# psweens/VAN-GAN

Hardware: AMD Instinct MI355X
Metric: train Mvoxels/s (VanGan.train_step, 128^3 bf16) (higher is better)
Workload: dtype bf16; 1 GPU; VanGan.train_step, 128x128x128 volumes, batch 1 per GPU (global 1), clDice on, disc noise+dropout on; parallelism=dp1

## Files before the change

### van_gan_amd/csrc/vg_loss.hip

```cpp
#include "vg_common.h"

static inline int lblocks(int64_t n, int per = 256) { int64_t b = (n + per - 1) / per; return (int)(b > 4095 ? 4095 : (b < 1 ? 1 : b)); }

__device__ __forceinline__ float block_sum(float v, float* sm) {
    v = wave_sum(v);
    const int lane = threadIdx.x & 63, wv = threadIdx.x >> 6;
    __syncthreads();
    if (lane == 0) sm[wv] = v;
    __syncthreads();
    float r = 0.f;
    for (int i = 0; i < (int)(blockDim.x >> 6); ++i) r += sm[i];
    return r;
}

__global__ void mm_init_kernel(float* mm4, int B) {
    const int b = blockIdx.x * blockDim.x + threadIdx.x;
    if (b < B) { mm4[b * 4] = INFINITY; mm4[b * 4 + 1] = -INFINITY; mm4[b * 4 + 2] = 0.f; mm4[b * 4 + 3] = 0.f; }
}
__device__ __forceinline__ void atomic_min_f(float* a, float v) {
    unsigned* ua = (unsigned*)a; unsigned old = *ua;
    while (v < __uint_as_float(old)) { const unsigned prev = atomicCAS(ua, old, __float_as_uint(v)); if (prev == old) break; old = prev; }
}
__device__ __forceinline__ void atomic_max_f(float* a, float v) {
    unsigned* ua = (unsigned*)a; unsigned old = *ua;
// ... 139 lines not shown
    if (threadIdx.x == 0) atomicAdd(acc, s);
}
extern "C" int vg_mse(const float* a, const float* b, int64_t n, float* acc, float gscale, float* gb, int accumulate,
                      vg_stream_t stream) {
    vg_begin();
    if (!a || !b || !acc || n < 1) return VG_EINVAL;
    hipLaunchKernelGGL(mse_kernel, dim3(lblocks(n, 1024) > 511 ? 511 : lblocks(n, 1024)), dim3(256), 0, (hipStream_t)stream, a, b, n, acc, gscale, gb,
                       accumulate);
    return vg_check_launch();
}
__global__ void mse_const_kernel(const void* x, int x_f32, float target, int64_t n, float* acc, float gscale, float* gx, int accum) {
    __shared__ float sm[4];
    float s = 0.f;
    for (int64_t i = (int64_t)blockIdx.x * blockDim.x + threadIdx.x; i < n; i += (int64_t)gridDim.x * blockDim.x) {
        const float v = x_f32 ? ((const float*)x)[i] : bf2f(((const bf16_t*)x)[i]);
        const float d = v - target;
        s += d * d;
        if (gx) { const float g = gscale * 2.f * d; gx[i] = accum ? gx[i] + g : g; }
    }
    s = block_sum(s, sm);
    if (threadIdx.x == 0) atomicAdd(acc, s);
}
extern "C" int vg_mse_const(const void* x, int x_f32, float target, int64_t n, float* acc, float gscale, float* gx,
                            int accumulate, vg_stream_t stream) {
    vg_begin();
    if (!x || !acc || n < 1) return VG_EINVAL;
    hipLaunchKernelGGL(mse_const_kernel, dim3(lblocks(n, 1024)), dim3(256), 0, (hipStream_t)stream, x, x_f32, target, n, acc,
                       gscale, gx, accumulate);
    return vg_check_launch();
}
template <int P>
__device__ __forceinline__ float lp_term(float d, float gscale, float& g) {
    if (P == 1) { g = d > 0.f ? gscale : (d < 0.f ? -gscale : 0.f); return fabsf(d); }
    if (P == 2) { g = gscale * 2.f * d; return d * d; }
    const float d2 = d * d;
    g = gscale * 4.f * (d2 * d);
    return d2 * d2;
}
template <int P>
__global__ __launch_bounds__(256) void lp_loss_kernel(const float* __restrict__ a, const float* __restrict__ b, int64_t n, float* acc, float gscale,
                                                      float* gb, int accum) {
    __shared__ float sm[4];
    float s = 0.f;
    const int64_t n4 = ((((uintptr_t)a | (uintptr_t)b | (uintptr_t)gb) & 15) == 0) ? n >> 2 : 0;
    for (int64_t i = (int64_t)blockIdx.x * blockDim.x + threadIdx.x; i < n4; i += (int64_t)gridDim.x * blockDim.x) {
        const f32x4 x = ((const f32x4*)a)[i], y = ((const f32x4*)b)[i];
        f32x4 g;
#pragma unroll
        for (int j = 0; j < 4; ++j) { float gj; s += lp_term<P>(y[j] - x[j], gscale, gj); g[j] = gj; }
        if (gb) { if (accum) g += ((const f32x4*)gb)[i]; ((f32x4*)gb)[i] = g; }
    }
    for (int64_t i = 4 * n4 + (int64_t)blockIdx.x * blockDim.x + threadIdx.x; i < n; i += (int64_t)gridDim.x * blockDim.x) {
        float g;
        s += lp_term<P>(b[i] - a[i], gscale, g);
        if (gb) gb[i] = accum ? gb[i] + g : g;
    }
    s = block_sum(s, sm);
    if (threadIdx.x == 0) atomicAdd(acc, s);
}
extern "C" int vg_lp_loss(const float* a, const float* b, int64_t n, int p, float* acc, float gscale, float* gb, int accumulate,
                          vg_stream_t stream) {
    vg_begin();
    if (!a || !b || !acc || n < 1 || (p != 1 && p != 2 && p != 4)) return VG_EINVAL;
    const dim3 grid(lblocks(n, 4096) > 511 ? 511 : lblocks(n, 4096));
    hipStream_t s = (hipStream_t)stream;
    if (p == 1) hipLaunchKernelGGL(lp_loss_kernel<1>, grid, dim3(256), 0, s, a, b, n, acc, gscale, gb, accumulate);
    else if (p == 2) hipLaunchKernelGGL(lp_loss_kernel<2>, grid, dim3(256), 0, s, a, b, n, acc, gscale, gb, accumulate);
    else hipLaunchKernelGGL(lp_loss_kernel<4>, grid, dim3(256), 0, s, a, b, n, acc, gscale, gb, accumulate);
    return vg_check_launch();
}
template <int KIND>
__device__ __forceinline__ float logit_term(float x, bool one, float& g) {
    const float e = expf(-fabsf(x));
    const float r = 1.f / (1.f + e);
    const float s = x >= 0.f ? r : e * r, c = x >= 0.f ? e * r : r;
    const float l1p = log1pf(e);
    const float sp = one ? fmaxf(-x, 0.f) + l1p : fmaxf(x, 0.f) + l1p;
    if (KIND == 0) { g = one ? -c : s; return sp; }
    if (one) { g = -(c * c * c) - 2.f * s * c * c * sp; return c * c * sp; }
    g = s * s * s + 2.f * s * s * c * sp;
    return s * s * sp;
}
template <int KIND, typename T>
__global__ __launch_bounds__(256) void logit_loss_kernel(const T* __restrict__ x, int one, int64_t n, float* acc, float gscale, float* gx, int accum) {
    __shared__ float sm[4];
    float s = 0.f;
    const int64_t n8 = ((((uintptr_t)x | (uintptr_t)gx) & 15) == 0) ? n >> 3 : 0;
    for (int64_t i = (int64_t)blockIdx.x * blockDim.x + threadIdx.x; i < n8; i += (int64_t)gridDim.x * blockDim.x) {
        float v[8], g[8];
        load8<T>(x + 8 * i, v);
#pragma unroll
        for (int j = 0; j < 8; ++j) { s += logit_term<KIND>(v[j], one != 0, g[j]); g[j] *= gscale; }
        if (gx) {
            if (accum) {
                float o[8]; load8<float>(gx + 8 * i, o);
#pragma unroll
                for (int j = 0; j < 8; ++j) g[j] += o[j];
            }
            store8<float>(gx + 8 * i, g);
        }
    }
    for (int64_t i = 8 * n8 + (int64_t)blockIdx.x * blockDim.x + threadIdx.x; i < n; i += (int64_t)gridDim.x * blockDim.x) {
        float g;
        s += logit_term<KIND>(ld1<T>(x + i), one != 0, g);
        g *= gscale;
        if (gx) gx[i] = accum ? gx[i] + g : g;
    }
    s = block_sum(s, sm);
    if (threadIdx.x == 0) atomicAdd(acc, s);
}
extern "C" int vg_logit_loss(const void* x, int x_f32, float target, int kind, int64_t n, float* acc, float gscale, float* gx,
                             int accumulate, vg_stream_t stream) {
    vg_begin();
    if (!x || !acc || n < 1 || (target != 0.f && target != 1.f) || (kind != 0 && kind != 1)) return VG_EINVAL;
    const dim3 grid(lblocks(n, 2048) > 255 ? 255 : lblocks(n, 2048));
    hipStream_t s = (hipStream_t)stream;
    const int one = target == 1.f;
#define VG_LOGIT_LAUNCH(K, T) hipLaunchKernelGGL((logit_loss_kernel<K, T>), grid, dim3(256), 0, s, (const T*)x, one, n, acc, gscale, gx, accumulate)
    if (kind == 0) { if (x_f32) VG_LOGIT_LAUNCH(0, float); else VG_LOGIT_LAUNCH(0, bf16_t); }
    else           { if (x_f32) VG_LOGIT_LAUNCH(1, float); else VG_LOGIT_LAUNCH(1, bf16_t); }
#undef VG_LOGIT_LAUNCH
    return vg_check_launch();
}
__global__ void dot_sums_kernel(const float* a, const float* b, int64_t n, float* sums3) {
    __shared__ float sm[4];
    float s0 = 0.f, s1 = 0.f, s2 = 0.f;
    const int64_t n4 = ((((uintptr_t)a | (uintptr_t)b) & 15) == 0) ? n >> 2 : 0;
    for (int64_t i = (int64_t)blockIdx.x * blockDim.x + threadIdx.x; i < n4; i += (int64_t)gridDim.x * blockDim.x) {
        const f32x4 x = ((const f32x4*)a)[i], y = ((const f32x4*)b)[i];
#pragma unroll
        for (int j = 0; j < 4; ++j) { s0 += x[j] * y[j]; s1 += x[j]; s2 += y[j]; }
    }
    for (int64_t i = 4 * n4 + (int64_t)blockIdx.x * blockDim.x + threadIdx.x; i < n; i += (int64_t)gridDim.x * blockDim.x) {
        const float x = a[i], y = b[i]; s0 += x * y; s1 += x; s2 += y;
    }
    s0 = block_sum(s0, sm); s1 = block_sum(s1, sm); s2 = block_sum(s2, sm);
    if (threadIdx.x == 0) { atomicAdd(&sums3[0], s0); atomicAdd(&sums3[1], s1); atomicAdd(&sums3[2], s2); }
}
extern "C" int vg_dot_sums(const float* a, const float* b, int64_t n, float* sums3, vg_stream_t stream) {
    vg_begin();
    if (!a || !b || !sums3 || n < 1) return VG_EINVAL;
    const int blocks = lblocks(n, 4096) > 255 ? 255 : lblocks(n, 4096);
    hipLaunchKernelGGL(dot_sums_kernel, dim3(blocks), dim3(256), 0, (hipStream_t)stream, a, b, n, sums3);
    return vg_check_launch();
}

__device__ __forceinline__ void gauss3(float* g) {
    const float e = expf(-0.5f * (1.f / 1.5f) * (1.f / 1.5f));
    const float s = 1.f + 2.f * e;
    g[0] = e / s; g[1] = 1.f / s; g[2] = e / s;
}
#define SSIM_C1 1e-4f
#define SSIM_C2 9e-4f
__global__ void ssim_fwd_kernel(const float* t, const float* p, int B, int D, int H, int W, float* acc, float* part) {
    __shared__ float sm[4];
    float g[3]; gauss3(g);
    const int64_t S = (int64_t)D * H * W, total = (int64_t)B * S;
    float loss = 0.f;
    for (int64_t i = (int64_t)blockIdx.x * blockDim.x + threadIdx.x; i < total; i += (int64_t)gridDim.x * blockDim.x) {
        const int w = (int)(i % W); int64_t r = i / W; const int h = (int)(r % H); r /= H; const int d = (int)(r % D); const int b = (int)(r / D);
        float mt = 0.f, mp = 0.f, ett = 0.f, epp = 0.f, etp = 0.f;
        for (int a = -1; a <= 1; ++a) { const int dd = d + a; if (dd < 0 || dd >= D) continue;
            for (int c = -1; c <= 1; ++c) { const int hh = h + c; if (hh < 0 || hh >= H) continue;
                for (int e = -1; e <= 1; ++e) { const int ww = w + e; if (ww < 0 || ww >= W) continue;
                    const float wt = g[a + 1] * g[c + 1] * g[e + 1];
                    const size_t j = (size_t)b * S + ((size_t)dd * H + hh) * W + ww;
                    const float tv = t[j], pv = p[j];
                    mt += wt * tv; mp += wt * pv; ett += wt * tv * tv; epp += wt * pv * pv; etp += wt * tv * pv;
                } } }
        const float stt = ett - mt * mt, spp = epp - mp * mp, stp = etp - mt * mp;
        const float A = 2.f * mt * mp + SSIM_C1, Bq = 2.f * stp + SSIM_C2;
        const float Cq = mt * mt + mp * mp + SSIM_C1, Dq = stt + spp + SSIM_C2;
        const float inv = 1.f / (Cq * Dq);
        const float ssim = A * Bq * inv;
        loss += 1.f - ssim;
        if (part) {
            const float dmu = (2.f * mt * Bq - 2.f * mt * A) * inv - ssim * (2.f * mp * Dq - 2.f * mp * Cq) * inv;
            const float depp = -ssim / Dq;
            const float detp = 2.f * A * inv;
            part[i] = -dmu; part[total + i] = -depp; part[2 * total + i] = -detp;
        }
    }
    loss = block_sum(loss, sm);
    if (threadIdx.x == 0) atomicAdd(acc, loss);
}
extern "C" int vg_ssim_fwd(const float* t, const float* p, int B, int D, int H, int W, float* acc, float* part,
                           vg_stream_t stream) {
    vg_begin();
    if (!t || !p || !acc || B < 1 || D < 1 || H < 1 || W < 1) return VG_EINVAL;
    const int blocks = lblocks((int64_t)B * D * H * W) > 1023 ? 1023 : lblocks((int64_t)B * D * H * W);
    hipLaunchKernelGGL(ssim_fwd_kernel, dim3(blocks), dim3(256), 0, (hipStream_t)stream, t, p, B, D, H, W, acc, part);
    return vg_check_launch();
}
__global__ void ssim_bwd_kernel(const float* t, const float* p, const float* part, int B, int D, int H, int W, float gscale,
                                float* gp, int accum) {
    float g[3]; gauss3(g);
    const int64_t S = (int64_t)D * H * W, total = (int64_t)B * S;
    for (int64_t i = (int64_t)blockIdx.x * blockDim.x + threadIdx.x; i < total; i += (int64_t)gridDim.x * blockDim.x) {
        const int w = (int)(i % W); int64_t r = i / W; const int h = (int)(r % H); r /= H; const int d = (int)(r % D); const int b = (int)(r / D);
        float f0 = 0.f, f1 = 0.f, f2 = 0.f;
        for (int a = -1; a <= 1; ++a) { const int dd = d + a; if (dd < 0 || dd >= D) continue;
            for (int c = -1; c <= 1; ++c) { const int hh = h + c; if (hh < 0 || hh >= H) continue;
                for (int e = -1; e <= 1; ++e) { const int ww = w + e; if (ww < 0 || ww >= W) continue;
                    const float wt = g[a + 1] * g[c + 1] * g[e + 1];
                    const size_t j = (size_t)b * S + ((size_t)dd * H + hh) * W + ww;
                    f0 += wt * part[j]; f1 += wt * part[total + j]; f2 += wt * part[2 * total + j];
                } } }
        const float v = gscale * (f0 + 2.f * p[i] * f1 + t[i] * f2);
        gp[i] = accum ? gp[i] + v : v;
    }
}
extern "C" int vg_ssim_bwd(const float* t, const float* p, const float* part, int B, int D, int H, int W, float gscale,
                           float* gp, int accumulate, vg_stream_t stream) {
    vg_begin();
    if (!t || !p || !part || !gp || B < 1) return VG_EINVAL;
    hipLaunchKernelGGL(ssim_bwd_kernel, dim3(lblocks((int64_t)B * D * H * W)), dim3(256), 0, (hipStream_t)stream, t, p, part, B, D, H, W,
                       gscale, gp, accumulate);
    return vg_check_launch();
}

#define SK_TW 32
#define SK_TH 8
#define SK_TD 8
template <bool ERODE>
__global__ __launch_bounds__(256) void skel_tile_kernel(const float* __restrict__ in, const float* __restrict__ imgj,
                                                        const float* __restrict__ prev, int D, int H, int W, float* __restrict__ out) {
    __shared__ float t[SK_TD + 2][SK_TH + 2][SK_TW + 2];
    const int tid = threadIdx.x;
    const int tiles_w = (W + SK_TW - 1) / SK_TW, tiles_h = (H + SK_TH - 1) / SK_TH;
    int bt = blockIdx.x;
    const int tw = bt % tiles_w; bt /= tiles_w;
    const int th = bt % tiles_h; const int td = bt / tiles_h;
    const int w0 = tw * SK_TW, h0 = th * SK_TH, d0 = td * SK_TD;
    const size_t vol = (size_t)blockIdx.y * D * H * W;
    const float fill = ERODE ? INFINITY : -INFINITY;
    constexpr int NH = (SK_TD + 2) * (SK_TH + 2) * (SK_TW + 2);
    for (int i = tid; i < NH; i += 256) {
        const int x = i % (SK_TW + 2); const int r = i / (SK_TW + 2);
        const int y = r % (SK_TH + 2), z = r / (SK_TH + 2);
        const int gw = w0 + x - 1, gh = h0 + y - 1, gd = d0 + z - 1;
        float v = fill;
        if (gw >= 0 && gw < W && gh >= 0 && gh < H && gd >= 0 && gd < D) v = in[vol + ((size_t)gd * H + gh) * W + gw];
        (&t[0][0][0])[i] = v;
    }
    __syncthreads();
    const int tx = tid & (SK_TW - 1), ty = tid >> 5;
    const int gw = w0 + tx, gh = h0 + ty;
    float p9[3], p5[3];
#pragma unroll
    for (int sl = 0; sl < SK_TD + 2; ++sl) {
        const float a00 = t[sl][ty][tx], a01 = t[sl][ty][tx + 1], a02 = t[sl][ty][tx + 2];
        const float a10 = t[sl][ty + 1][tx], a11 = t[sl][ty + 1][tx + 1], a12 = t[sl][ty + 1][tx + 2];
        const float a20 = t[sl][ty + 2][tx], a21 = t[sl][ty + 2][tx + 1], a22 = t[sl][ty + 2][tx + 2];
        float plus, full;
        if (ERODE) {
            plus = fminf(fminf(fminf(a01, a21), fminf(a10, a12)), a11);
            full = fminf(plus, fminf(fminf(a00, a02), fminf(a20, a22)));
        } else {
            plus = fmaxf(fmaxf(fmaxf(a01, a21), fmaxf(a10, a12)), a11);
            full = fmaxf(plus, fmaxf(fmaxf(a00, a02), fmaxf(a20, a22)));
        }
        p9[sl % 3] = full; p5[sl % 3] = plus;
        if (sl >= 2) {
            const int gd = d0 + sl - 2;
            const int c = (sl - 1) % 3, lo = (sl - 2) % 3, hi = sl % 3;
            const float nb = ERODE ? fminf(p9[c], fminf(p5[lo], p5[hi])) : fmaxf(p9[c], fmaxf(p9[lo], p9[hi]));
            if (gw < W && gh < H && gd < D) {
                const size_t o = vol + ((size_t)gd * H + gh) * W + gw;
                if (ERODE) out[o] = nb;
                else {
                    const float delta = fmaxf(imgj[o] - nb, 0.f);
                    if (prev) { const float sp = prev[o]; out[o] = sp + fmaxf(delta - sp * delta, 0.f); }
                    else out[o] = delta;
                }
            }
        }
    }
}
template <bool AUX>
__global__ __launch_bounds__(256) void skel_chain_kernel(const float* __restrict__ imgs, int64_t n, int iters, int D, int H, int W,
                                                         float* __restrict__ skels, float* __restrict__ deltas, unsigned char* __restrict__ codes) {
    __shared__ float t[SK_TD + 2][SK_TH + 2][SK_TW + 2];
    const int tid = threadIdx.x;
    const int tiles_w = (W + SK_TW - 1) / SK_TW, tiles_h = (H + SK_TH - 1) / SK_TH;
    int bt = blockIdx.x;
    const int tw = bt % tiles_w; bt /= tiles_w;
    const int th = bt % tiles_h; const int td = bt / tiles_h;
    const int w0 = tw * SK_TW, h0 = th * SK_TH, d0 = td * SK_TD;
    const size_t vol = (size_t)blockIdx.y * D * H * W;
    constexpr int NH = (SK_TD + 2) * (SK_TH + 2) * (SK_TW + 2);
    const int tx = tid & (SK_TW - 1), ty = tid >> 5;
    const int gw = w0 + tx, gh = h0 + ty;
    const bool col_ok = gw < W && gh < H;
    float cen[SK_TD], sk[SK_TD];
#pragma unroll
    for (int k = 0; k < SK_TD; ++k) {
        const int gd = d0 + k;
        cen[k] = (col_ok && gd < D) ? imgs[vol + ((size_t)gd * H + gh) * W + gw] : 0.f;
        sk[k] = 0.f;
    }
    for (int j = 0; j <= iters; ++j) {
        const float* __restrict__ in = imgs + (size_t)(j + 1) * n;
        __syncthreads();
        for (int i = tid; i < NH; i += 256) {
            const int x = i % (SK_TW + 2); const int r = i / (SK_TW + 2);
            const int y = r % (SK_TH + 2), z = r / (SK_TH + 2);
            const int qw = w0 + x - 1, qh = h0 + y - 1, qd = d0 + z - 1;
            float v = -INFINITY;
            if (qw >= 0 && qw < W && qh >= 0 && qh < H && qd >= 0 && qd < D) v = in[vol + ((size_t)qd * H + qh) * W + qw];
            (&t[0][0][0])[i] = v;
        }
        __syncthreads();
        float* __restrict__ out = skels + (size_t)j * n;
        float p9[3]; int k9[3];
#pragma unroll
        for (int sl = 0; sl < SK_TD + 2; ++sl) {
            const float a00 = t[sl][ty][tx], a01 = t[sl][ty][tx + 1], a02 = t[sl][ty][tx + 2];
            const float a10 = t[sl][ty + 1][tx], a11 = t[sl][ty + 1][tx + 1], a12 = t[sl][ty + 1][tx + 2];
            const float a20 = t[sl][ty + 2][tx], a21 = t[sl][ty + 2][tx + 1], a22 = t[sl][ty + 2][tx + 2];
            if (AUX) {
                float m = a00; int k = 0;
                if (a01 > m) { m = a01; k = 1; } if (a02 > m) { m = a02; k = 2; }
                if (a10 > m) { m = a10; k = 3; } if (a11 > m) { m = a11; k = 4; } if (a12 > m) { m = a12; k = 5; }
                if (a20 > m) { m = a20; k = 6; } if (a21 > m) { m = a21; k = 7; } if (a22 > m) { m = a22; k = 8; }
                p9[sl % 3] = m; k9[sl % 3] = k;
            } else {
                const float plus = fmaxf(fmaxf(fmaxf(a01, a21), fmaxf(a10, a12)), a11);
                p9[sl % 3] = fmaxf(plus, fmaxf(fmaxf(a00, a02), fmaxf(a20, a22)));
            }
            if (sl >= 2) {
                const int k = sl - 2, gd = d0 + k;
                const float nb = fmaxf(p9[(sl - 1) % 3], fmaxf(p9[(sl - 2) % 3], p9[sl % 3]));
                const float delta = fmaxf(cen[k] - nb, 0.f);
                const float sp = sk[k];
                sk[k] = j ? sp + fmaxf(delta - sp * delta, 0.f) : delta;
                if (col_ok && gd < D) {
                    const size_t o = vol + ((size_t)gd * H + gh) * W + gw;
                    out[o] = sk[k];
                    if (AUX) {
                        float best = p9[(sl - 2) % 3]; int code = k9[(sl - 2) % 3];
                        if (p9[(sl - 1) % 3] > best) { best = p9[(sl - 1) % 3]; code = 9 + k9[(sl - 1) % 3]; }
                        if (p9[sl % 3] > best) { best = p9[sl % 3]; code = 18 + k9[sl % 3]; }
                        deltas[(size_t)j * n + o] = delta; codes[(size_t)j * n + o] = (unsigned char)code;
                    }
                }
            }
        }
#pragma unroll
        for (int k = 0; k < SK_TD; ++k) cen[k] = t[k + 1][ty + 1][tx + 1];
    }
}
__device__ __forceinline__ int64_t sk_off(int code, int H, int W) {
    const int a = code / 9, r = code - a * 9, b = r / 3, c = r - b * 3;
    return ((int64_t)(a - 1) * H + (b - 1)) * W + (c - 1);
}
#define SK_TILE_ORIGIN()                                                                                    \
    const int tiles_w = (W + SK_TW - 1) / SK_TW, tiles_h = (H + SK_TH - 1) / SK_TH;                           \
    int bt_ = blockIdx.x; const int tw_ = bt_ % tiles_w; bt_ /= tiles_w;                                      \
    const int th_ = bt_ % tiles_h, td_ = bt_ / tiles_h;                                                       \
    const int w0 = tw_ * SK_TW, h0 = th_ * SK_TH, d0 = td_ * SK_TD;                                           \
    const size_t vol = (size_t)blockIdx.y * D * H * W;                                                        \
    const int tx = tid & (SK_TW - 1), ty = tid >> 5; const int gw = w0 + tx, gh = h0 + ty;

template <int E>
__device__ __forceinline__ void erode_stage(const float* __restrict__ src, float* __restrict__ dst, int w0, int h0, int d0, int D, int H, int W,
                                            size_t vol, float* __restrict__ out, int tid) {
    constexpr int DD = SK_TD + 2 * E, DH = SK_TH + 2 * E, DW = SK_TW + 2 * E;
    constexpr int SH = DH + 2, SW = DW + 2;
    for (int col = tid; col < DH * DW; col += 256) {
        const int y = col / DW, x = col - y * DW;
        const int gh = h0 - E + y, gw = w0 - E + x;
        const bool col_in = gh >= 0 && gh < H && gw >= 0 && gw < W;
        const bool col_tile = y >= E && y < E + SK_TH && x >= E && x < E + SK_TW;
        float p9[3], p5[3];
#pragma unroll
        for (int sl = 0; sl < DD + 2; ++sl) {
            const float* r0 = src + (sl * SH + y) * SW + x;
            const float* r1 = r0 + SW; const float* r2 = r1 + SW;
            const float a00 = r0[0], a01 = r0[1], a02 = r0[2], a10 = r1[0], a11 = r1[1], a12 = r1[2], a20 = r2[0], a21 = r2[1], a22 = r2[2];
            const float plus = fminf(fminf(fminf(a01, a21), fminf(a10, a12)), a11);
            p9[sl % 3] = fminf(plus, fminf(fminf(a00, a02), fminf(a20, a22))); p5[sl % 3] = plus;
            if (sl >= 2) {
                const int z = sl - 2, gd = d0 - E + z;
                const float nb = fminf(p9[(sl - 1) % 3], fminf(p5[(sl - 2) % 3], p5[sl % 3]));
                const bool in = col_in && gd >= 0 && gd < D;
                if (E > 0) dst[(z * DH + y) * DW + x] = in ? nb : INFINITY;
                if (in && col_tile && z >= E && z < E + SK_TD) out[vol + ((size_t)gd * H + gh) * W + gw] = nb;
            }
        }
    }
}
template <int K>
__global__ __launch_bounds__(256) void erode_multi_kernel(const float* __restrict__ in, int D, int H, int W, int64_t n, float* __restrict__ outs,
                                                          float* __restrict__ copy0) {
    extern __shared__ float sk_lds[];
    constexpr int XD = SK_TD + 2 * K, XH = SK_TH + 2 * K, XW = SK_TW + 2 * K;
    float* A = sk_lds; float* Bf = sk_lds + XD * XH * XW;
    const int tid = threadIdx.x;
    SK_TILE_ORIGIN()
    (void)tx; (void)ty; (void)gw; (void)gh;
    for (int i = tid; i < XD * XH * XW; i += 256) {
        const int x = i % XW; const int r = i / XW; const int y = r % XH, z = r / XH;
        const int qw = w0 - K + x, qh = h0 - K + y, qd = d0 - K + z;
        float v = INFINITY;
        if (qw >= 0 && qw < W && qh >= 0 && qh < H && qd >= 0 && qd < D) {
            const size_t o = vol + ((size_t)qd * H + qh) * W + qw;
            v = in[o];
            if (copy0 && x >= K && x < K + SK_TW && y >= K && y < K + SK_TH && z >= K && z < K + SK_TD) copy0[o] = v;
        }
        A[i] = v;
    }
    __syncthreads();
    erode_stage<K - 1>(A, Bf, w0, h0, d0, D, H, W, vol, outs, tid);
    if constexpr (K >= 2) { __syncthreads(); erode_stage<K - 2>(Bf, A, w0, h0, d0, D, H, W, vol, outs + n, tid); }
    if constexpr (K >= 3) { __syncthreads(); erode_stage<K - 3>(A, Bf, w0, h0, d0, D, H, W, vol, outs + 2 * n, tid); }
    if constexpr (K >= 4) { __syncthreads(); erode_stage<K - 4>(Bf, A, w0, h0, d0, D, H, W, vol, outs + 3 * n, tid); }
}
template <int K>
static void launch_erode_multi(const float* in, int D, int H, int W, int64_t n, float* outs, float* copy0, dim3 grid, hipStream_t s) {
    constexpr int XD = SK_TD + 2 * K, XH = SK_TH + 2 * K, XW = SK_TW + 2 * K;
    constexpr int lds = (XD * XH * XW + (XD - 2) * (XH - 2) * (XW - 2)) * 4;
    static bool attr = false;
    if (!attr) { (void)hipFuncSetAttribute((const void*)erode_multi_kernel<K>, hipFuncAttributeMaxDynamicSharedMemorySize, VG_LDS_LIMIT); attr = true; }
    hipLaunchKernelGGL(erode_multi_kernel<K>, grid, dim3(256), lds, s, in, D, H, W, n, outs, copy0);
}
static dim3 skel_grid(int B, int D, int H, int W) {
    return dim3(((W + SK_TW - 1) / SK_TW) * ((H + SK_TH - 1) / SK_TH) * ((D + SK_TD - 1) / SK_TD), B);
}
__device__ __forceinline__ void sk_load_tile(float (&t)[SK_TD + 2][SK_TH + 2][SK_TW + 2], const float* __restrict__ in, size_t vol,
                                             int w0, int h0, int d0, int D, int H, int W, float fill, int tid) {
    constexpr int NH = (SK_TD + 2) * (SK_TH + 2) * (SK_TW + 2);
    for (int i = tid; i < NH; i += 256) {
        const int x = i % (SK_TW + 2); const int r = i / (SK_TW + 2);
        const int y = r % (SK_TH + 2), z = r / (SK_TH + 2);
        const int gw = w0 + x - 1, gh = h0 + y - 1, gd = d0 + z - 1;
        float v = fill;
        if (gw >= 0 && gw < W && gh >= 0 && gh < H && gd >= 0 && gd < D) v = in[vol + ((size_t)gd * H + gh) * W + gw];
        (&t[0][0][0])[i] = v;
    }
}
__global__ __launch_bounds__(256) void skel_bwd_local_kernel(const float* __restrict__ imgj, const float* __restrict__ imgj1,
                                                             const float* __restrict__ prev, int D, int H, int W,
                                                             float* gs, float* dimgj, float* dimgj1) {
    __shared__ float t[SK_TD + 2][SK_TH + 2][SK_TW + 2];
    const int tid = threadIdx.x;
    SK_TILE_ORIGIN()
    sk_load_tile(t, imgj1, vol, w0, h0, d0, D, H, W, -INFINITY, tid);
    __syncthreads();
    if (gw >= W || gh >= H) return;
    float m9[3]; int k9[3];
#pragma unroll
    for (int sl = 0; sl < SK_TD + 2; ++sl) {
        const float a00 = t[sl][ty][tx], a01 = t[sl][ty][tx + 1], a02 = t[sl][ty][tx + 2];
        const float a10 = t[sl][ty + 1][tx], a11 = t[sl][ty + 1][tx + 1], a12 = t[sl][ty + 1][tx + 2];
        const float a20 = t[sl][ty + 2][tx], a21 = t[sl][ty + 2][tx + 1], a22 = t[sl][ty + 2][tx + 2];
        float m = a00; int k = 0;
        if (a01 > m) { m = a01; k = 1; } if (a02 > m) { m = a02; k = 2; }
        if (a10 > m) { m = a10; k = 3; } if (a11 > m) { m = a11; k = 4; } if (a12 > m) { m = a12; k = 5; }
        if (a20 > m) { m = a20; k = 6; } if (a21 > m) { m = a21; k = 7; } if (a22 > m) { m = a22; k = 8; }
        m9[sl % 3] = m; k9[sl % 3] = k;
        if (sl < 2) continue;
        const int gd = d0 + sl - 2;
        if (gd >= D) continue;
        const size_t i = vol + ((size_t)gd * H + gh) * W + gw;
        float dil = m9[(sl - 2) % 3]; int code = k9[(sl - 2) % 3];
        if (m9[(sl - 1) % 3] > dil) { dil = m9[(sl - 1) % 3]; code = 9 + k9[(sl - 1) % 3]; }
        if (m9[sl % 3] > dil) { dil = m9[sl % 3]; code = 18 + k9[sl % 3]; }
        const float raw = imgj[i] - dil;
        const float delta = fmaxf(raw, 0.f);
        const float g = gs[i];
        float ddelta;
        if (prev) {
            const float sp = prev[i];
            const float u = delta - sp * delta;
            const float dr = u > 0.f ? g : 0.f;
            ddelta = dr * (1.f - sp);
            gs[i] = g - dr * delta;
        } else ddelta = g;
        const float e = raw > 0.f ? ddelta : 0.f;
        if (e != 0.f) { dimgj[i] += e; atomicAdd(&dimgj1[(int64_t)i + sk_off(code, H, W)], -e); }
    }
}
__global__ __launch_bounds__(256) void erode_bwd_kernel(const float* __restrict__ imgj, float* __restrict__ dimgj1,
                                                        int D, int H, int W, float* dimgj) {
    __shared__ float t[SK_TD + 2][SK_TH + 2][SK_TW + 2];
    const int tid = threadIdx.x;
    SK_TILE_ORIGIN()
    sk_load_tile(t, imgj, vol, w0, h0, d0, D, H, W, INFINITY, tid);
    __syncthreads();
    if (gw >= W || gh >= H) return;
    float vC[3], vR[3], vF[3]; int iC[3], iR[3], iF[3];
#pragma unroll
    for (int sl = 0; sl < SK_TD + 2; ++sl) {
        const float a00 = t[sl][ty][tx], a01 = t[sl][ty][tx + 1], a02 = t[sl][ty][tx + 2];
        const float a10 = t[sl][ty + 1][tx], a11 = t[sl][ty + 1][tx + 1], a12 = t[sl][ty + 1][tx + 2];
        const float a20 = t[sl][ty + 2][tx], a21 = t[sl][ty + 2][tx + 1], a22 = t[sl][ty + 2][tx + 2];
        { float m = a01; int k = 0; if (a11 < m) { m = a11; k = 1; } if (a21 < m) { m = a21; k = 2; } vC[sl % 3] = m; iC[sl % 3] = k; }
        { float m = a10; int k = 0; if (a11 < m) { m = a11; k = 1; } if (a12 < m) { m = a12; k = 2; } vR[sl % 3] = m; iR[sl % 3] = k; }
        { float m = a00; int k = 0;
          if (a01 < m) { m = a01; k = 1; } if (a02 < m) { m = a02; k = 2; }
          if (a10 < m) { m = a10; k = 3; } if (a11 < m) { m = a11; k = 4; } if (a12 < m) { m = a12; k = 5; }
          if (a20 < m) { m = a20; k = 6; } if (a21 < m) { m = a21; k = 7; } if (a22 < m) { m = a22; k = 8; }
          vF[sl % 3] = m; iF[sl % 3] = k; }
        if (sl < 2) continue;
        const int gd = d0 + sl - 2;
        if (gd >= D) continue;
        const size_t i = vol + ((size_t)gd * H + gh) * W + gw;
        const float g = dimgj1[i];
        if (g == 0.f) continue;
        dimgj1[i] = 0.f;
        const int lo = (sl - 2) % 3, c = (sl - 1) % 3, hi = sl % 3;
        float best = vC[lo]; int code = iC[lo] * 3 + 1;
        if (vC[c] < best) { best = vC[c]; code = 9 + iC[c] * 3 + 1; }
        if (vC[hi] < best) { best = vC[hi]; code = 18 + iC[hi] * 3 + 1; }
        if (vR[lo] < best) { best = vR[lo]; code = 3 + iR[lo]; }
        if (vR[c] < best) { best = vR[c]; code = 12 + iR[c]; }
        if (vR[hi] < best) { best = vR[hi]; code = 21 + iR[hi]; }
        if (vF[c] < best) { best = vF[c]; code = 9 + iF[c]; }
        atomicAdd(&dimgj[(int64_t)i + sk_off(code, H, W)], g);
    }
}

__global__ __launch_bounds__(256) void skel_erode_code_kernel(const float* __restrict__ in, int D, int H, int W, float* __restrict__ out,
                                                              unsigned char* __restrict__ codes) {
    __shared__ float t[SK_TD + 2][SK_TH + 2][SK_TW + 2];
    const int tid = threadIdx.x;
    SK_TILE_ORIGIN()
    sk_load_tile(t, in, vol, w0, h0, d0, D, H, W, INFINITY, tid);
    __syncthreads();
    float vC[3], vR[3], vF[3]; int iC[3], iR[3], iF[3];
#pragma unroll
    for (int sl = 0; sl < SK_TD + 2; ++sl) {
        const float a00 = t[sl][ty][tx], a01 = t[sl][ty][tx + 1], a02 = t[sl][ty][tx + 2];
        const float a10 = t[sl][ty + 1][tx], a11 = t[sl][ty + 1][tx + 1], a12 = t[sl][ty + 1][tx + 2];
        const float a20 = t[sl][ty + 2][tx], a21 = t[sl][ty + 2][tx + 1], a22 = t[sl][ty + 2][tx + 2];
        { float m = a01; int k = 0; if (a11 < m) { m = a11; k = 1; } if (a21 < m) { m = a21; k = 2; } vC[sl % 3] = m; iC[sl % 3] = k; }
        { float m = a10; int k = 0; if (a11 < m) { m = a11; k = 1; } if (a12 < m) { m = a12; k = 2; } vR[sl % 3] = m; iR[sl % 3] = k; }
        { float m = a00; int k = 0;
          if (a01 < m) { m = a01; k = 1; } if (a02 < m) { m = a02; k = 2; }
          if (a10 < m) { m = a10; k = 3; } if (a11 < m) { m = a11; k = 4; } if (a12 < m) { m = a12; k = 5; }
          if (a20 < m) { m = a20; k = 6; } if (a21 < m) { m = a21; k = 7; } if (a22 < m) { m = a22; k = 8; }
          vF[sl % 3] = m; iF[sl % 3] = k; }
        if (sl >= 2) {
            const int gd = d0 + sl - 2;
            const int lo = (sl - 2) % 3, c = (sl - 1) % 3, hi = sl % 3;
            float best = vC[lo]; int code = iC[lo] * 3 + 1;
            if (vC[c] < best) { best = vC[c]; code = 9 + iC[c] * 3 + 1; }
            if (vC[hi] < best) { best = vC[hi]; code = 18 + iC[hi] * 3 + 1; }
            if (vR[lo] < best) { best = vR[lo]; code = 3 + iR[lo]; }
            if (vR[c] < best) { best = vR[c]; code = 12 + iR[c]; }
            if (vR[hi] < best) { best = vR[hi]; code = 21 + iR[hi]; }
            if (vF[c] < best) { best = vF[c]; code = 9 + iF[c]; }
            if (gw < W && gh < H && gd < D) {
                const size_t o = vol + ((size_t)gd * H + gh) * W + gw;
                out[o] = best; codes[o] = (unsigned char)code;
            }
        }
    }
}

template <int V> __device__ __forceinline__ void sk_ldf(const float* p, int64_t q, float* o) {
    if constexpr (V == 4) { const f32x4 v = ((const f32x4*)p)[q]; o[0] = v[0]; o[1] = v[1]; o[2] = v[2]; o[3] = v[3]; } else o[0] = p[q];
}
template <int V> __device__ __forceinline__ void sk_stf(float* p, int64_t q, const float* o) {
    if constexpr (V == 4) ((f32x4*)p)[q] = (f32x4){o[0], o[1], o[2], o[3]}; else p[q] = o[0];
}
template <int V> __device__ __forceinline__ void sk_ldc(const unsigned char* p, int64_t q, int* o) {
    if constexpr (V == 4) { const unsigned w = ((const unsigned*)p)[q]; o[0] = w & 255; o[1] = (w >> 8) & 255; o[2] = (w >> 16) & 255; o[3] = w >> 24; }
    else o[0] = p[q];
}
template <int V>
__global__ __launch_bounds__(256) void skel_bwd_stream_kernel(const float* __restrict__ d_in, const unsigned char* __restrict__ codeN,
                                                              float* d_acc, float* d_out, int out_accumulate,
                                                              const float* __restrict__ delta, const unsigned char* __restrict__ codeM,
                                                              const float* __restrict__ prev, const float* gs_in, float* gs_out,
                                                              int64_t n, int H, int W) {
    const int64_t nv = n / V;
    for (int64_t q = (int64_t)blockIdx.x * blockDim.x + threadIdx.x; q < nv; q += (int64_t)gridDim.x * blockDim.x) {
        const int64_t i0 = q * V;
        float g_in[V], dl[V], sp[V], g[V]; int cn[V], cm[V];
        if (d_in) { sk_ldf<V>(d_in, q, g_in); sk_ldc<V>(codeN, q, cn); }
        if (delta) { sk_ldf<V>(delta, q, dl); sk_ldf<V>(gs_in, q, g); sk_ldc<V>(codeM, q, cm); if (prev) sk_ldf<V>(prev, q, sp); }
        if (d_in) {
#pragma unroll
            for (int v = 0; v < V; ++v)
                if (g_in[v] != 0.f) atomicAdd(&d_acc[i0 + v + sk_off(cn[v], H, W)], g_in[v]);
        }
        if (delta) {
            float e[V], gn[V];
            bool changed = false;
#pragma unroll
            for (int v = 0; v < V; ++v) {
                float ddelta; gn[v] = g[v];
                if (prev) {
                    const float u = dl[v] - sp[v] * dl[v];
                    const float dr = u > 0.f ? g[v] : 0.f;
                    ddelta = dr * (1.f - sp[v]);
                    gn[v] = g[v] - dr * dl[v];
                } else ddelta = g[v];
                e[v] = dl[v] > 0.f ? ddelta : 0.f;
                changed |= gn[v] != g[v];
                if (e[v] != 0.f) atomicAdd(&d_acc[i0 + v + sk_off(cm[v], H, W)], -e[v]);
            }
            if (prev && (changed || gs_in != gs_out)) sk_stf<V>(gs_out, q, gn);
            if (out_accumulate) {
                float o[V]; sk_ldf<V>(d_out, q, o);
#pragma unroll
                for (int v = 0; v < V; ++v) e[v] += o[v];
            }
            sk_stf<V>(d_out, q, e);
        }
    }
}
extern "C" int vg_soft_skel_fwd(const float* img, int B, int D, int H, int W, int iters, float* imgs, float* skels, void* aux,
                                vg_stream_t stream) {
    vg_begin();
    if (!img || !imgs || !skels || B < 1 || iters < 0) return VG_EINVAL;
    hipStream_t s = (hipStream_t)stream;
    const int64_t n = (int64_t)B * D * H * W;
    const dim3 grid = skel_grid(B, D, H, W);
    const int multi = vg_tune("SKEL_MULTI", 2);
    float* deltas = (float*)aux;
    unsigned char* codeM = aux ? (unsigned char*)(deltas + (size_t)(iters + 1) * n) : nullptr;
    unsigned char* codeN = aux ? codeM + (size_t)(iters + 1) * n : nullptr;
    if (aux) {
        if (hipMemcpyAsync(imgs, img, n * sizeof(float), hipMemcpyDeviceToDevice, s) != hipSuccess) return VG_ELAUNCH;
        for (int j = 0; j <= iters; ++j)
            hipLaunchKernelGGL(skel_erode_code_kernel, grid, dim3(256), 0, s, (const float*)(imgs + j * n), D, H, W, imgs + (j + 1) * n, codeN + (size_t)j * n);
    } else if (multi > 1) {
        for (int j = 0; j <= iters;) {
            const int left = iters + 1 - j;
            const float* in = j ? imgs + j * n : img;
            float* c0 = j ? nullptr : imgs;
            if (left >= 4 && multi >= 4) { launch_erode_multi<4>(in, D, H, W, n, imgs + (j + 1) * n, c0, grid, s); j += 4; }
            else if (left >= 2) { launch_erode_multi<2>(in, D, H, W, n, imgs + (j + 1) * n, c0, grid, s); j += 2; }
            else { launch_erode_multi<1>(in, D, H, W, n, imgs + (j + 1) * n, c0, grid, s); j += 1; }
        }
    } else {
        if (hipMemcpyAsync(imgs, img, n * sizeof(float), hipMemcpyDeviceToDevice, s) != hipSuccess) return VG_ELAUNCH;
        for (int j = 0; j <= iters; ++j)
            hipLaunchKernelGGL(skel_tile_kernel<true>, grid, dim3(256), 0, s, imgs + j * n, (const float*)nullptr, (const float*)nullptr,
                               D, H, W, imgs + (j + 1) * n);
    }
    if (aux) {
        hipLaunchKernelGGL(skel_chain_kernel<true>, grid, dim3(256), 0, s, (const float*)imgs, n, iters, D, H, W, skels, deltas, codeM);
        return vg_check_launch();
    }
    if (vg_tune("SKEL_CHAIN", 1)) {
        hipLaunchKernelGGL(skel_chain_kernel<false>, grid, dim3(256), 0, s, (const float*)imgs, n, iters, D, H, W, skels, (float*)nullptr, (unsigned char*)nullptr);
        return vg_check_launch();
    }
    for (int j = 0; j <= iters; ++j)
        hipLaunchKernelGGL(skel_tile_kernel<false>, grid, dim3(256), 0, s, imgs + (j + 1) * n, imgs + j * n,
                           j ? skels + (j - 1) * n : (const float*)nullptr, D, H, W, skels + j * n);
    return vg_check_launch();
}

extern "C" int vg_soft_skel_bwd(const float* imgs, const float* skels, const float* gskel, int B, int D, int H, int W,
                                int iters, float* work, float* gimg, const void* aux, vg_stream_t stream) {
    vg_begin();
    if (!imgs || !skels || !gskel || !work || !gimg || B < 1 || iters < 0) return VG_EINVAL;
// ... 170 lines not shown
```

Baseline: 123.2 Mvoxels/s.

## Batch halo and stencil loads into registers before shared-memory commit

Replaces the strided halo-fill loops in the skeleton/erode kernels with a templated scheme that issues all global loads up front into registers with clamped addresses and an inside-bitmask, then commits to LDS, so many loads are in flight at once. Per-column operands (imgj, prev, gs, dimgj) are prefetched before the barrier, and the iterative skeleton kernel prefetches the next level's halo while computing the current one. SSIM fwd/bwd stencils now load all 27 neighbors unconditionally with clamped indices and mask the accumulation instead of branching. The cost is higher register pressure and possible lower occupancy, plus extra redundant loads at the borders.

```diff
diff --git a/van_gan_amd/csrc/vg_loss.hip b/van_gan_amd/csrc/vg_loss.hip
--- a/van_gan_amd/csrc/vg_loss.hip
+++ b/van_gan_amd/csrc/vg_loss.hip
@@ -315,22 +315,40 @@
 }
 #define SSIM_C1 1e-4f
 #define SSIM_C2 9e-4f
-__global__ void ssim_fwd_kernel(const float* t, const float* p, int B, int D, int H, int W, float* acc, float* part) {
+__global__ __launch_bounds__(256) void ssim_fwd_kernel(const float* t, const float* p, int B, int D, int H, int W, float* acc, float* part) {
     __shared__ float sm[4];
     float g[3]; gauss3(g);
     const int64_t S = (int64_t)D * H * W, total = (int64_t)B * S;
     float loss = 0.f;
     for (int64_t i = (int64_t)blockIdx.x * blockDim.x + threadIdx.x; i < total; i += (int64_t)gridDim.x * blockDim.x) {
         const int w = (int)(i % W); int64_t r = i / W; const int h = (int)(r % H); r /= H; const int d = (int)(r % D); const int b = (int)(r / D);
+        float tv[27], pv[27];
+        unsigned inside = 0;
+        const float* tb = t + (size_t)b * S; const float* pb = p + (size_t)b * S;
+#pragma unroll
+        for (int a = -1; a <= 1; ++a) { const int dd = d + a, cd = min(max(dd, 0), D - 1);
+#pragma unroll
+            for (int c = -1; c <= 1; ++c) { const int hh = h + c, ch = min(max(hh, 0), H - 1);
+#pragma unroll
+                for (int e = -1; e <= 1; ++e) { const int ww = w + e, cw = min(max(ww, 0), W - 1);
+                    const int k = ((a + 1) * 3 + (c + 1)) * 3 + (e + 1);
+                    const size_t j = ((size_t)cd * H + ch) * W + cw;
+                    tv[k] = ld_global(tb + j); pv[k] = ld_global(pb + j);
+                    inside |= (unsigned)((cd == dd) & (ch == hh) & (cw == ww)) << k;
+                } } }
         float mt = 0.f, mp = 0.f, ett = 0.f, epp = 0.f, etp = 0.f;
-        for (int a = -1; a <= 1; ++a) { const int dd = d + a; if (dd < 0 || dd >= D) continue;
-            for (int c = -1; c <= 1; ++c) { const int hh = h + c; if (hh < 0 || hh >= H) continue;
-                for (int e = -1; e <= 1; ++e) { const int ww = w + e; if (ww < 0 || ww >= W) continue;
-                    const float wt = g[a + 1] * g[c + 1] * g[e + 1];
-                    const size_t j = (size_t)b * S + ((size_t)dd * H + hh) * W + ww;
-                    const float tv = t[j], pv = p[j];
-                    mt += wt * tv; mp += wt * pv; ett += wt * tv * tv; epp += wt * pv * pv; etp += wt * tv * pv;
-                } } }
+#pragma unroll
+        for (int a = 0; a < 3; ++a)
+#pragma unroll
+            for (int c = 0; c < 3; ++c)
+#pragma unroll
+                for (int e = 0; e < 3; ++e) {
+                    const int k = (a * 3 + c) * 3 + e;
+                    const bool in = (inside >> k) & 1;
+                    const float wt = g[a] * g[c] * g[e];
+                    mt = in ? mt + wt * tv[k] : mt; mp = in ? mp + wt * pv[k] : mp;
+                    ett = in ? ett + wt * tv[k] * tv[k] : ett; epp = in ? epp + wt * pv[k] * pv[k] : epp; etp = in ? etp + wt * tv[k] * pv[k] : etp;
+                }
         const float stt = ett - mt * mt, spp = epp - mp * mp, stp = etp - mt * mp;
         const float A = 2.f * mt * mp + SSIM_C1, Bq = 2.f * stp + SSIM_C2;
         const float Cq = mt * mt + mp * mp + SSIM_C1, Dq = stt + spp + SSIM_C2;
@@ -355,22 +373,41 @@
     hipLaunchKernelGGL(ssim_fwd_kernel, dim3(blocks), dim3(256), 0, (hipStream_t)stream, t, p, B, D, H, W, acc, part);
     return vg_check_launch();
 }
-__global__ void ssim_bwd_kernel(const float* t, const float* p, const float* part, int B, int D, int H, int W, float gscale,
+__global__ __launch_bounds__(256) void ssim_bwd_kernel(const float* t, const float* p, const float* part, int B, int D, int H, int W, float gscale,
                                 float* gp, int accum) {
     float g[3]; gauss3(g);
     const int64_t S = (int64_t)D * H * W, total = (int64_t)B * S;
     for (int64_t i = (int64_t)blockIdx.x * blockDim.x + threadIdx.x; i < total; i += (int64_t)gridDim.x * blockDim.x) {
         const int w = (int)(i % W); int64_t r = i / W; const int h = (int)(r % H); r /= H; const int d = (int)(r % D); const int b = (int)(r / D);
+        float q0[27], q1[27], q2[27];
+        unsigned inside = 0;
+        const float* pb = part + (size_t)b * S;
+#pragma unroll
+        for (int a = -1; a <= 1; ++a) { const int dd = d + a, cd = min(max(dd, 0), D - 1);
+#pragma unroll
+            for (int c = -1; c <= 1; ++c) { const int hh = h + c, ch = min(max(hh, 0), H - 1);
+#pragma unroll
+                for (int e = -1; e <= 1; ++e) { const int ww = w + e, cw = min(max(ww, 0), W - 1);
+                    const int k = ((a + 1) * 3 + (c + 1)) * 3 + (e + 1);
+                    const size_t j = ((size_t)cd * H + ch) * W + cw;
+                    q0[k] = ld_global(pb + j); q1[k] = ld_global(pb + total + j); q2[k] = ld_global(pb + 2 * total + j);
+                    inside |= (unsigned)((cd == dd) & (ch == hh) & (cw == ww)) << k;
+                } } }
+        const float pi = ld_global(p + i), ti = ld_global(t + i), old = ld_global(gp + i);
         float f0 = 0.f, f1 = 0.f, f2 = 0.f;
-        for (int a = -1; a <= 1; ++a) { const int dd = d + a; if (dd < 0 || dd >= D) continue;
-            for (int c = -1; c <= 1; ++c) { const int hh = h + c; if (hh < 0 || hh >= H) continue;
-                for (int e = -1; e <= 1; ++e) { const int ww = w + e; if (ww < 0 || ww >= W) continue;
-                    const float wt = g[a + 1] * g[c + 1] * g[e + 1];
-                    const size_t j = (size_t)b * S + ((size_t)dd * H + hh) * W + ww;
-                    f0 += wt * part[j]; f1 += wt * part[total + j]; f2 += wt * part[2 * total + j];
-                } } }
-        const float v = gscale * (f0 + 2.f * p[i] * f1 + t[i] * f2);
-        gp[i] = accum ? gp[i] + v : v;
+#pragma unroll
+        for (int a = 0; a < 3; ++a)
+#pragma unroll
+            for (int c = 0; c < 3; ++c)
+#pragma unroll
+                for (int e = 0; e < 3; ++e) {
+                    const int k = (a * 3 + c) * 3 + e;
+                    const bool in = (inside >> k) & 1;
+                    const float wt = g[a] * g[c] * g[e];
+                    f0 = in ? f0 + wt * q0[k] : f0; f1 = in ? f1 + wt * q1[k] : f1; f2 = in ? f2 + wt * q2[k] : f2;
+                }
+        const float v = gscale * (f0 + 2.f * pi * f1 + ti * f2);
+        gp[i] = accum ? old + v : v;
     }
 }
 extern "C" int vg_ssim_bwd(const float* t, const float* p, const float* part, int B, int D, int H, int W, float gscale,
@@ -385,6 +422,74 @@
 #define SK_TW 32
 #define SK_TH 8
 #define SK_TD 8
+template <int E> struct SkHalo {
+    static constexpr int XD = SK_TD + 2 * E, XH = SK_TH + 2 * E, XW = SK_TW + 2 * E;
+    static constexpr int P = XH * XW, FP = P / 256, R = P % 256, NA = XD * FP, NB = (XD * R + 255) / 256;
+    static constexpr int N = XD * P, NR = NA + NB;
+    static_assert(FP >= 1 && FP <= 4 && R > 0 && NB <= 12 && XD <= 16, "bit layout of the inside mask");
+    static __device__ __forceinline__ int index(int k, int tid) {
+        if (k < NA) return (k / FP) * P + tid + 256 * (k % FP);
+        const int i = min(tid + 256 * (k - NA), XD * R - 1);
+        const int z = i / R;
+        return z * P + 256 * FP + (i - z * R);
+    }
+    static __device__ __forceinline__ bool inside(uint32_t mask, int k) {
+        if (k < NA) return (mask >> (k % FP)) & (mask >> (16 + k / FP)) & 1;
+        return (mask >> (4 + k - NA)) & 1;
+    }
+};
+__device__ __forceinline__ const float* sk_uniform(const float* p) {
+    const uint64_t a = (uint64_t)(uintptr_t)p;
+    const uint32_t lo = __builtin_amdgcn_readfirstlane((uint32_t)a), hi = __builtin_amdgcn_readfirstlane((uint32_t)(a >> 32));
+    return (const float*)(uintptr_t)(((uint64_t)hi << 32) | lo);
+}
+template <int E>
+__device__ __forceinline__ uint32_t sk_halo_request(float (&v)[SkHalo<E>::NR], const float* __restrict__ in, size_t vol,
+                                                    int w0, int h0, int d0, int D, int H, int W, int tid) {
+    using G = SkHalo<E>;
+    const float* base = in + vol;
+    uint32_t mask = 0;
+    size_t offA[G::FP];
+#pragma unroll
+    for (int q = 0; q < G::FP; ++q) {
+        const int e = tid + 256 * q;
+        const int y = e / G::XW, x = e - y * G::XW;
+        const int gw = w0 - E + x, gh = h0 - E + y;
+        const int cw = min(max(gw, 0), W - 1), ch = min(max(gh, 0), H - 1);
+        mask |= (uint32_t)((cw == gw) & (ch == gh)) << q;
+        offA[q] = (size_t)ch * W + cw;
+    }
+#pragma unroll
+    for (int z = 0; z < G::XD; ++z) {
+        const int gd = d0 - E + z, cd = min(max(gd, 0), D - 1);
+        mask |= (uint32_t)(cd == gd) << (16 + z);
+        const float* plane = sk_uniform(base + (size_t)cd * H * W);
+#pragma unroll
+        for (int q = 0; q < G::FP; ++q) v[z * G::FP + q] = ld_global(plane + offA[q]);
+    }
+#pragma unroll
+    for (int m = 0; m < G::NB; ++m) {
+        const int i = G::index(G::NA + m, tid);
+        const int x = i % G::XW; const int r = i / G::XW;
+        const int y = r % G::XH, z = r / G::XH;
+        const int gw = w0 - E + x, gh = h0 - E + y, gd = d0 - E + z;
+        const int cw = min(max(gw, 0), W - 1), ch = min(max(gh, 0), H - 1), cd = min(max(gd, 0), D - 1);
+        mask |= (uint32_t)((cw == gw) & (ch == gh) & (cd == gd)) << (4 + m);
+        v[G::NA + m] = ld_global(base + ((size_t)cd * H + ch) * W + cw);
+    }
+    return mask;
+}
+template <int E>
+__device__ __forceinline__ void sk_halo_commit(float* __restrict__ t, const float (&v)[SkHalo<E>::NR], uint32_t mask, float fill, int tid) {
+    using G = SkHalo<E>;
+#pragma unroll
+    for (int k = 0; k < G::NR; ++k) t[G::index(k, tid)] = G::inside(mask, k) ? v[k] : fill;
+}
+__device__ __forceinline__ void sk_col_request(float (&v)[SK_TD], const float* p, size_t vol, int gw, int gh, int d0, int D, int H, int W) {
+    const int cw = min(gw, W - 1), ch = min(gh, H - 1);
+#pragma unroll
+    for (int k = 0; k < SK_TD; ++k) v[k] = ld_global(p + vol + ((size_t)min(d0 + k, D - 1) * H + ch) * W + cw);
+}
 template <bool ERODE>
 __global__ __launch_bounds__(256) void skel_tile_kernel(const float* __restrict__ in, const float* __restrict__ imgj,
                                                         const float* __restrict__ prev, int D, int H, int W, float* __restrict__ out) {
@@ -397,18 +502,16 @@
     const int w0 = tw * SK_TW, h0 = th * SK_TH, d0 = td * SK_TD;
     const size_t vol = (size_t)blockIdx.y * D * H * W;
     const float fill = ERODE ? INFINITY : -INFINITY;
-    constexpr int NH = (SK_TD + 2) * (SK_TH + 2) * (SK_TW + 2);
-    for (int i = tid; i < NH; i += 256) {
-        const int x = i % (SK_TW + 2); const int r = i / (SK_TW + 2);
-        const int y = r % (SK_TH + 2), z = r / (SK_TH + 2);
-        const int gw = w0 + x - 1, gh = h0 + y - 1, gd = d0 + z - 1;
-        float v = fill;
-        if (gw >= 0 && gw < W && gh >= 0 && gh < H && gd >= 0 && gd < D) v = in[vol + ((size_t)gd * H + gh) * W + gw];
-        (&t[0][0][0])[i] = v;
-    }
-    __syncthreads();
     const int tx = tid & (SK_TW - 1), ty = tid >> 5;
     const int gw = w0 + tx, gh = h0 + ty;
+    float hv[SkHalo<1>::NR], cj[SK_TD], cp[SK_TD];
+    const uint32_t inside = sk_halo_request<1>(hv, in, vol, w0, h0, d0, D, H, W, tid);
+    if (!ERODE) {
+        sk_col_request(cj, imgj, vol, gw, gh, d0, D, H, W);
+        sk_col_request(cp, prev ? prev : imgj, vol, gw, gh, d0, D, H, W);
+    }
+    sk_halo_commit<1>(&t[0][0][0], hv, inside, fill, tid);
+    __syncthreads();
     float p9[3], p5[3];
 #pragma unroll
     for (int sl = 0; sl < SK_TD + 2; ++sl) {
@@ -432,8 +535,8 @@
                 const size_t o = vol + ((size_t)gd * H + gh) * W + gw;
                 if (ERODE) out[o] = nb;
                 else {
-                    const float delta = fmaxf(imgj[o] - nb, 0.f);
-                    if (prev) { const float sp = prev[o]; out[o] = sp + fmaxf(delta - sp * delta, 0.f); }
+                    const float delta = fmaxf(cj[sl - 2] - nb, 0.f);
+                    if (prev) { const float sp = cp[sl - 2]; out[o] = sp + fmaxf(delta - sp * delta, 0.f); }
                     else out[o] = delta;
                 }
             }
@@ -451,29 +554,20 @@
     const int th = bt % tiles_h; const int td = bt / tiles_h;
     const int w0 = tw * SK_TW, h0 = th * SK_TH, d0 = td * SK_TD;
     const size_t vol = (size_t)blockIdx.y * D * H * W;
-    constexpr int NH = (SK_TD + 2) * (SK_TH + 2) * (SK_TW + 2);
     const int tx = tid & (SK_TW - 1), ty = tid >> 5;
     const int gw = w0 + tx, gh = h0 + ty;
     const bool col_ok = gw < W && gh < H;
-    float cen[SK_TD], sk[SK_TD];
-#pragma unroll
-    for (int k = 0; k < SK_TD; ++k) {
-        const int gd = d0 + k;
-        cen[k] = (col_ok && gd < D) ? imgs[vol + ((size_t)gd * H + gh) * W + gw] : 0.f;
-        sk[k] = 0.f;
-    }
+    float cen[SK_TD], sk[SK_TD], hv[SkHalo<1>::NR];
+    const uint32_t inside = sk_halo_request<1>(hv, imgs + n, vol, w0, h0, d0, D, H, W, tid);
+    sk_col_request(cen, imgs, vol, gw, gh, d0, D, H, W);
+#pragma unroll
+    for (int k = 0; k < SK_TD; ++k) sk[k] = 0.f;
     for (int j = 0; j <= iters; ++j) {
-        const float* __restrict__ in = imgs + (size_t)(j + 1) * n;
+        if (AUX && j > 0) sk_halo_request<1>(hv, imgs + (size_t)(j + 1) * n, vol, w0, h0, d0, D, H, W, tid);
         __syncthreads();
-        for (int i = tid; i < NH; i += 256) {
-            const int x = i % (SK_TW + 2); const int r = i / (SK_TW + 2);
-            const int y = r % (SK_TH + 2), z = r / (SK_TH + 2);
-            const int qw = w0 + x - 1, qh = h0 + y - 1, qd = d0 + z - 1;
-            float v = -INFINITY;
-            if (qw >= 0 && qw < W && qh >= 0 && qh < H && qd >= 0 && qd < D) v = in[vol + ((size_t)qd * H + qh) * W + qw];
-            (&t[0][0][0])[i] = v;
-        }
+        sk_halo_commit<1>(&t[0][0][0], hv, inside, -INFINITY, tid);
         __syncthreads();
+        if (!AUX && j < iters) sk_halo_request<1>(hv, imgs + (size_t)(j + 2) * n, vol, w0, h0, d0, D, H, W, tid);
         float* __restrict__ out = skels + (size_t)j * n;
         float p9[3]; int k9[3];
 #pragma unroll
@@ -562,16 +656,17 @@
     const int tid = threadIdx.x;
     SK_TILE_ORIGIN()
     (void)tx; (void)ty; (void)gw; (void)gh;
-    for (int i = tid; i < XD * XH * XW; i += 256) {
-        const int x = i % XW; const int r = i / XW; const int y = r % XH, z = r / XH;
-        const int qw = w0 - K + x, qh = h0 - K + y, qd = d0 - K + z;
-        float v = INFINITY;
-        if (qw >= 0 && qw < W && qh >= 0 && qh < H && qd >= 0 && qd < D) {
-            const size_t o = vol + ((size_t)qd * H + qh) * W + qw;
-            v = in[o];
-            if (copy0 && x >= K && x < K + SK_TW && y >= K && y < K + SK_TH && z >= K && z < K + SK_TD) copy0[o] = v;
-        }
-        A[i] = v;
+    float hv[SkHalo<K>::NR];
+    const uint32_t inside = sk_halo_request<K>(hv, in, vol, w0, h0, d0, D, H, W, tid);
+    sk_halo_commit<K>(A, hv, inside, INFINITY, tid);
+    if (copy0) {
+#pragma unroll
+        for (int k = 0; k < SkHalo<K>::NR; ++k) {
+            const int i = SkHalo<K>::index(k, tid);
+            const int x = i % XW; const int r = i / XW; const int y = r % XH, z = r / XH;
+            if (SkHalo<K>::inside(inside, k) && x >= K && x < K + SK_TW && y >= K && y < K + SK_TH && z >= K && z < K + SK_TD)
+                copy0[vol + ((size_t)(d0 - K + z) * H + (h0 - K + y)) * W + (w0 - K + x)] = hv[k];
+        }
     }
     __syncthreads();
     erode_stage<K - 1>(A, Bf, w0, h0, d0, D, H, W, vol, outs, tid);
@@ -592,15 +687,9 @@
 }
 __device__ __forceinline__ void sk_load_tile(float (&t)[SK_TD + 2][SK_TH + 2][SK_TW + 2], const float* __restrict__ in, size_t vol,
                                              int w0, int h0, int d0, int D, int H, int W, float fill, int tid) {
-    constexpr int NH = (SK_TD + 2) * (SK_TH + 2) * (SK_TW + 2);
-    for (int i = tid; i < NH; i += 256) {
-        const int x = i % (SK_TW + 2); const int r = i / (SK_TW + 2);
-        const int y = r % (SK_TH + 2), z = r / (SK_TH + 2);
-        const int gw = w0 + x - 1, gh = h0 + y - 1, gd = d0 + z - 1;
-        float v = fill;
-        if (gw >= 0 && gw < W && gh >= 0 && gh < H && gd >= 0 && gd < D) v = in[vol + ((size_t)gd * H + gh) * W + gw];
-        (&t[0][0][0])[i] = v;
-    }
+    float hv[SkHalo<1>::NR];
+    const uint32_t inside = sk_halo_request<1>(hv, in, vol, w0, h0, d0, D, H, W, tid);
+    sk_halo_commit<1>(&t[0][0][0], hv, inside, fill, tid);
 }
 __global__ __launch_bounds__(256) void skel_bwd_local_kernel(const float* __restrict__ imgj, const float* __restrict__ imgj1,
                                                              const float* __restrict__ prev, int D, int H, int W,
@@ -608,7 +697,13 @@
     __shared__ float t[SK_TD + 2][SK_TH + 2][SK_TW + 2];
     const int tid = threadIdx.x;
     SK_TILE_ORIGIN()
-    sk_load_tile(t, imgj1, vol, w0, h0, d0, D, H, W, -INFINITY, tid);
+    float hv[SkHalo<1>::NR], cj[SK_TD], cg[SK_TD], cp[SK_TD], ca[SK_TD];
+    const uint32_t inside = sk_halo_request<1>(hv, imgj1, vol, w0, h0, d0, D, H, W, tid);
+    sk_col_request(cj, imgj, vol, gw, gh, d0, D, H, W);
+    sk_col_request(cg, gs, vol, gw, gh, d0, D, H, W);
+    sk_col_request(cp, prev ? prev : imgj, vol, gw, gh, d0, D, H, W);
+    sk_col_request(ca, dimgj, vol, gw, gh, d0, D, H, W);
+    sk_halo_commit<1>(&t[0][0][0], hv, inside, -INFINITY, tid);
     __syncthreads();
     if (gw >= W || gh >= H) return;
     float m9[3]; int k9[3];
@@ -629,19 +724,19 @@
         float dil = m9[(sl - 2) % 3]; int code = k9[(sl - 2) % 3];
         if (m9[(sl - 1) % 3] > dil) { dil = m9[(sl - 1) % 3]; code = 9 + k9[(sl - 1) % 3]; }
         if (m9[sl % 3] > dil) { dil = m9[sl % 3]; code = 18 + k9[sl % 3]; }
-        const float raw = imgj[i] - dil;
+        const float raw = cj[sl - 2] - dil;
         const float delta = fmaxf(raw, 0.f);
-        const float g = gs[i];
+        const float g = cg[sl - 2];
         float ddelta;
         if (prev) {
-            const float sp = prev[i];
+            const float sp = cp[sl - 2];
             const float u = delta - sp * delta;
             const float dr = u > 0.f ? g : 0.f;
             ddelta = dr * (1.f - sp);
             gs[i] = g - dr * delta;
         } else ddelta = g;
         const float e = raw > 0.f ? ddelta : 0.f;
-        if (e != 0.f) { dimgj[i] += e; atomicAdd(&dimgj1[(int64_t)i + sk_off(code, H, W)], -e); }
+        if (e != 0.f) { dimgj[i] = ca[sl - 2] + e; atomicAdd(&dimgj1[(int64_t)i + sk_off(code, H, W)], -e); }
     }
 }
 __global__ __launch_bounds__(256) void erode_bwd_kernel(const float* __restrict__ imgj, float* __restrict__ dimgj1,
@@ -649,7 +744,10 @@
     __shared__ float t[SK_TD + 2][SK_TH + 2][SK_TW + 2];
     const int tid = threadIdx.x;
     SK_TILE_ORIGIN()
-    sk_load_tile(t, imgj, vol, w0, h0, d0, D, H, W, INFINITY, tid);
+    float hv[SkHalo<1>::NR], cg[SK_TD];
+    const uint32_t inside = sk_halo_request<1>(hv, imgj, vol, w0, h0, d0, D, H, W, tid);
+    sk_col_request(cg, dimgj1, vol, gw, gh, d0, D, H, W);
+    sk_halo_commit<1>(&t[0][0][0], hv, inside, INFINITY, tid);
     __syncthreads();
     if (gw >= W || gh >= H) return;
     float vC[3], vR[3], vF[3]; int iC[3], iR[3], iF[3];
@@ -669,7 +767,7 @@
         const int gd = d0 + sl - 2;
         if (gd >= D) continue;
         const size_t i = vol + ((size_t)gd * H + gh) * W + gw;
-        const float g = dimgj1[i];
+        const float g = cg[sl - 2];
         if (g == 0.f) continue;
         dimgj1[i] = 0.f;
         const int lo = (sl - 2) % 3, c = (sl - 1) % 3, hi = sl % 3;
```

Measured after the change: 124.8 Mvoxels/s (median of 6 runs). +1.3%, better.
